# jfjlaros/HUMID

Hardware: AMD Instinct MI355X
Metric: reads/sec deduplicated, 10M PE150 UMI=8 d=1 (higher is better)
Workload: dtype u64; 1 GPU; 10000000 reads/GPU x 1 GPU (one shuffled read set of 10000000 reads, sliced by input order), PE150 UMI=8 in header -> 24-nt packed words (8+8+8), d=1, directional clustering; synthetic molecules=N/4, family 1+Geom(3), p_sub=1e-3, p_N=1e-4; reads_per_gpu=10000000, word_nt=24, distance=1, method=directional

## Files before the change

humid_amd/csrc/humid_hip.hip:

```cpp
#include "pipeline.hip.h"
#include "kernels_best.hip.h"
#include "kernels_consensus.hip.h"

static std::string g_err;
extern "C" __attribute__((visibility("hidden"))) void humid_set_global_error(const char *text) { g_err = text ? text : ""; }

extern "C" {

uint32_t humid_abi_version(void) { return HUMID_ABI_VERSION; }

int humid_device_count(void) {
  int n = 0;
  if (hipGetDeviceCount(&n) != hipSuccess) return 0;
  return n;
}

const char *humid_last_error(const humid_ctx *ctx) { return ctx ? ctx->err.c_str() : g_err.c_str(); }

int humid_ctx_create(humid_ctx **out, int device, void *stream) {
  humid_ctx *c = nullptr;
  if (!out) return fail(nullptr, HUMID_E_INVALID, "out is null");
  *out = nullptr;
  int ndev = 0;
  hipError_t e = hipGetDeviceCount(&ndev);
// ... 134 lines not shown
  }
  if (strcmp(key, "records8") == 0) {
    c->use_rec8 = value != 0;
    return HUMID_OK;
  }
  if (strcmp(key, "compact_graph") == 0) {
    c->use_compact = value != 0;
    return HUMID_OK;
  }
  if (strcmp(key, "group_buckets") == 0) {
    c->group_buckets = value != 0;
    return HUMID_OK;
  }
  if (strcmp(key, "fused_search") == 0) {
    c->fused_search = value != 0;
    return HUMID_OK;
  }
  if (strcmp(key, "padded_partition") == 0) {
    c->pt_padded = value != 0;
    return HUMID_OK;
  }
  if (strcmp(key, "force_comm") == 0) {
    c->force_comm = value != 0;
    return HUMID_OK;
  }
  if (strcmp(key, "bucket_walk") == 0) {
    if (value < 0 || value > (1 << 24)) return fail(c, HUMID_E_INVALID, "bucket_walk must be 0 (no limit) .. 2^24");
    c->walk_max = (u32)value;
    return HUMID_OK;
  }
// ... 824 lines not shown
```

humid_amd/csrc/kernels_cgraph.hip.h:

```cpp
#ifndef HUMID_KERNELS_CGRAPH_HIP_H
#define HUMID_KERNELS_CGRAPH_HIP_H

#include "common.hip.h"
#include "kernels_graph.hip.h"
#include "kernels_cluster.hip.h"

#define ER_REGIONS 64u
#define ER_STRIDE 32u
struct EdgeRegs {
  u64 *e;
  u32 cap_r;
  u32 *cur;
  const u64 *far;
  u32 n_far;
};
__device__ __forceinline__ u32 er_count(const EdgeRegs &er, u32 r) {
  if (r == ER_REGIONS) return er.n_far;
  const u32 c = er.cur[r * ER_STRIDE];
  return c < er.cap_r ? c : er.cap_r;
}
__device__ __forceinline__ u64 *er_at(const EdgeRegs &er, u32 r, u32 k) {
  return r == ER_REGIONS ? (u64 *)er.far + k : er.e + (size_t)r * er.cap_r + k;
}

// ... 31 lines not shown
static __global__ void __launch_bounds__(256)
k_bits_blocks(const u32 *__restrict__ bits, u32 n_blk, u32 *__restrict__ cnt) {
  HUMID_GUARD_LAST_VGPR();
  const u32 b = blockIdx.x * blockDim.x + threadIdx.x;
  if (b > n_blk) return;
  if (b == n_blk) { cnt[b] = 0; return; }
  const uint4 *p = (const uint4 *)(bits + 8 * (size_t)b);
  const uint4 x = p[0], y = p[1];
  cnt[b] = (u32)(__popc(x.x) + __popc(x.y) + __popc(x.z) + __popc(x.w) + __popc(y.x) + __popc(y.y) + __popc(y.z) + __popc(y.w));
}

#define ZERO_MAX 8
struct ZeroList {
  u32 *p[ZERO_MAX];
  u32 n[ZERO_MAX];
};
static __global__ void __launch_bounds__(256)
k_zero_many(ZeroList z) {
  HUMID_GUARD_LAST_VGPR();
  const u32 stride = gridDim.x * blockDim.x;
#pragma unroll
  for (u32 q = 0; q < ZERO_MAX; q++) {
    u32 *p = z.p[q];
    const u32 n = z.n[q];
    for (u32 i = blockIdx.x * blockDim.x + threadIdx.x; i < n; i += stride) p[i] = 0;
  }
}

#define PA_PPT 4u

template <class WT>
struct WordsGlobal {
  const WT *W;
  __device__ __forceinline__ WT operator()(u32 j) const { return W[j]; }
};
struct IdxSelf { __device__ __forceinline__ u32 operator()(u32 j) const { return j; } };
struct IdxGlobal {
  const u32 *V;
  __device__ __forceinline__ u32 operator()(u32 j) const { return V[j]; }
};
template <class WT>
// ... 176 lines not shown
  HUMID_GUARD_LAST_VGPR();
  const u32 r = blockIdx.y;
  const u32 n_r = er_count(er, r);
  for (u32 k = blockIdx.x * blockDim.x + threadIdx.x; k < n_r; k += gridDim.x * blockDim.x) {
    u64 *slot = er_at(er, r, k);
    const u64 e = *slot;
    const u32 a = br_rank(br, (u32)(e >> 32)), b = br_rank(br, (u32)e);
    *slot = ((u64)a << 32) | b;
    atomicAdd(&deg[a], 1u);
    atomicAdd(&deg[b], 1u);
    if (joins_for_clustering(join_by_count ? ncnt : (const u32 *)nullptr, a, b)) uf_union(parent, a, b);
  }
}

static __global__ void __launch_bounds__(256)
k_fill_and_stats(EdgeRegs er, const u32 *__restrict__ off, u32 *cur, u32 *__restrict__ idx, u32 *__restrict__ regions_max, u32 gx,
                 const u32 *__restrict__ deg, u32 *P, u32 n, u32 *csize, const u32 *__restrict__ n_dev, u32 r_first) {
  HUMID_GUARD_LAST_VGPR();
  const u32 nf = gx * (ER_REGIONS + 1 - r_first);
  if (blockIdx.x >= nf) {
    const u32 u = (blockIdx.x - nf) * blockDim.x + threadIdx.x;
    if (n_dev && *n_dev < n) n = *n_dev;
    if (u >= n || deg[u] == 0) return;
    const u32 root = uf_find(P, u);
    P[u] = root;
    atomicAdd(&csize[root], 1u);
    return;
  }
  const u32 bx = blockIdx.x % gx, r = r_first + blockIdx.x / gx;
  if (regions_max && blockIdx.x == 0 && threadIdx.x < 64) {
// ... 52 lines not shown
  if (ia >= n_ids || ib >= n_ids || ia == ib) { cpairs[k] = 0; return; }
  const u32 a = br_rank(br, ia), b = br_rank(br, ib);
  const u32 ca = (u32)r.y, cb = (u32)(r.y >> 32);
  cpairs[k] = ((u64)a << 32) | b;
  ncnt[a] = ca;
  ncnt[b] = cb;
  atomicAdd(&deg[a], 1u);
  atomicAdd(&deg[b], 1u);
  if (!join_by_count || at_least_double(ca, cb) || at_least_double(cb, ca)) uf_union(parent, a, b);
}

template <bool MAXIMUM>
__global__ void __launch_bounds__(256)
k_cg_trivial(const u32 *__restrict__ P, const u32 *__restrict__ csize, const u32 *__restrict__ m_dev, const u32 *__restrict__ cnt,
             const u32 *__restrict__ off, const u32 *__restrict__ idx, u32 *cl_of, u32 *maxleaf, u64 *cl_size, ull *ctr,
             u32 *__restrict__ small_roots) {
  HUMID_GUARD_LAST_VGPR();
  __shared__ u32 lds[4];
  __shared__ u32 lroots[CC_ROOTS], lroots_n, lroots_base;
  if (threadIdx.x == 0) lroots_n = 0;
  __syncthreads();
  const u32 n = *m_dev;
  const u32 lane = threadIdx.x & 63;
  u32 mb = 0, round = 0;
  for (u32 a0 = blockIdx.x * blockDim.x; a0 < n; a0 += gridDim.x * blockDim.x) {
    const u32 a = a0 + threadIdx.x;
    bool small_root = false;
    if (a < n) {
      const u32 root = P[a];
      const u32 members = csize[root];
      if (members > SMALL_COMP) { mb++; cl_of[a] = 0; }
      else if (members > 2) { small_root = root == a; cl_of[a] = 0; }
      else if (members == 1) { cl_of[a] = a + 1; maxleaf[a] = a; cl_size[a] = cnt[a]; }
      else if (root == a) {
        u32 b = a;
        for (u32 k = off[a]; k < off[a + 1]; k++) {
          const u32 nb = idx[k];
          if (P[nb] == root) { b = nb; break; }
        }
        const u64 ca = cnt[a], cb = cnt[b];
        if (MAXIMUM) {
          cl_of[a] = a + 1; cl_of[b] = a + 1;
          maxleaf[a] = (cb > ca) ? b : a;
          cl_size[a] = ca + cb;
        } else if (at_least_double(cb, ca)) {
          cl_of[a] = a + 1; cl_of[b] = a + 1;
          maxleaf[a] = b;
          cl_size[a] = ca + cb;
        } else if (at_least_double(ca, cb)) {
          cl_of[a] = a + 1; cl_of[b] = a + 1;
          maxleaf[a] = a;
          cl_size[a] = ca + cb;
        } else {
          cl_of[a] = a + 1; maxleaf[a] = a; cl_size[a] = ca;
          cl_of[b] = b + 1; maxleaf[b] = b; cl_size[b] = cb;
        }
      }
    }
    const u64 bm = __ballot(small_root);
    if (bm) {
      u32 base = 0;
      if (lane == 0) base = atomicAdd(&lroots_n, (u32)__popcll(bm));
      base = __shfl(base, 0);
      if (small_root) lroots[base + (u32)__popcll(bm & ((1ull << lane) - 1ull))] = a;
    }
    if ((++round & (CC_ROOTS / 256u - 1u)) == 0) {
      __syncthreads();
      const u32 cntl = lroots_n;
      if (cntl) {
        if (threadIdx.x == 0) lroots_base = (u32)atomicAdd(&ctr[CTR_SMALLROOTS], (ull)cntl);
// ... 75 lines not shown
```

humid_amd/csrc/kernels_cluster.hip.h:

```cpp
#ifndef HUMID_KERNELS_CLUSTER_HIP_H
#define HUMID_KERNELS_CLUSTER_HIP_H

#include "common.hip.h"
#include "kernels_graph.hip.h"
#include "kernels_count.hip.h"

#define MAX_CLIMB 40u

template <bool MAXIMUM, class MemberAt, class St>
__device__ __forceinline__ void cluster_one_component(MemberAt member_at, u32 n_members,
                                                      const u32 *__restrict__ cnt,
                                                      const u32 *__restrict__ off,
                                                      const u32 *__restrict__ idx, u32 *cl_of,
                                                      u32 *maxleaf, u64 *cl_size, St st) {
  for (u32 m = 0; m < n_members; m++) {
    const u32 u = member_at(m);
    if (cl_of[u] != 0) continue;
    const u32 label = u + 1;
    u32 start = u;
    u32 best = u;
    u32 bestc = 0;
    if (!MAXIMUM) {
      u32 leaf = u;
      u32 k = off[leaf], kend = off[leaf + 1];
// ... 248 lines not shown
    u32 m = k;
    while (m > 0 && mem[m - 1] > x) { mem[m] = mem[m - 1]; m--; }
    mem[m] = x;
  }
  cluster_one_component<MAXIMUM>([&](u32 m) { return mem[m]; }, nm, cnt, off, idx, cl_of, maxleaf, cl_size, st);
}

struct LdsColumn {
  u32 *base;
  __device__ __forceinline__ u32 &operator[](u32 i) const { return base[i * 64u]; }
};
template <bool MAXIMUM>
__global__ void __launch_bounds__(64)
k_cluster_small_lds(const u32 *__restrict__ roots, const ull *__restrict__ ctr, const u32 *__restrict__ P,
                    const u32 *__restrict__ csize, u32 n, const u32 *__restrict__ cnt, const u32 *__restrict__ off,
                    const u32 *__restrict__ idx, u32 *cl_of, u32 *maxleaf, u64 *cl_size) {
  HUMID_GUARD_LAST_VGPR();
  __shared__ u32 lmem[SMALL_COMP][64];
  __shared__ u32 lst[2 * SMALL_COMP][64];
  const u32 t = blockIdx.x * blockDim.x + threadIdx.x;
  if (t >= (u32)ctr[CTR_SMALLROOTS]) return;
  const u32 u = roots[t];
  if (u >= n) return;
  const u32 target = csize[u];
  if (target > SMALL_COMP || target <= 2) return;
  const LdsColumn mem{&lmem[0][threadIdx.x]}, st{&lst[0][threadIdx.x]};
  u32 nm = 1;
  mem[0] = u;
  for (u32 q = 0; q < nm && nm < target; q++) {
    const u32 v = mem[q];
    for (u32 k = off[v]; k < off[v + 1] && nm < target; k++) {
      const u32 nb = idx[k];
      bool seen = P[nb] != u;
      for (u32 j = 0; j < nm; j++) seen |= (mem[j] == nb);
      if (!seen) { mem[nm] = nb; nm++; }
    }
  }
  for (u32 k = 1; k < nm; k++) {
    const u32 x = mem[k];
    u32 m = k;
    while (m > 0 && mem[m - 1] > x) { mem[m] = mem[m - 1]; m--; }
    mem[m] = x;
  }
  cluster_one_component<MAXIMUM>([&](u32 m) { return mem[m]; }, nm, cnt, off, idx, cl_of, maxleaf, cl_size, st);
}

static __global__ void k_creator_flags(const u32 *__restrict__ cl_of, u32 n, u32 *flag) {
  HUMID_GUARD_LAST_VGPR();
  u32 u = blockIdx.x * blockDim.x + threadIdx.x;
  if (u < n) flag[u] = (cl_of[u] == u + 1) ? 1u : 0u;
}

static __global__ void k_finalize_nodes(const u32 *__restrict__ cl_of, const u32 *__restrict__ pos,
                                 const u32 *__restrict__ maxleaf, u32 n, u32 *__restrict__ cid,
                                 u8 *__restrict__ ismax, const u32 *__restrict__ s_first,
                                 const u32 *__restrict__ s_slot, u64 *__restrict__ slot_out) {
  HUMID_GUARD_LAST_VGPR();
  u32 u = blockIdx.x * blockDim.x + threadIdx.x;
  if (u >= n) return;
// ... 33 lines not shown
```

humid_amd/csrc/pipeline.hip.h:

```cpp
#ifndef HUMID_PIPELINE_HIP_H
#define HUMID_PIPELINE_HIP_H

#include <fcntl.h>
#include <sys/mman.h>
#include <sys/stat.h>
#include <unistd.h>

#include <atomic>
#include <cerrno>
#include <chrono>
#include <type_traits>
#include <utility>

#include "common.hip.h"
#include "prims.hip.h"
#include "kernels_count.hip.h"
#include "kernels_part.hip.h"
#include "kernels_part8.hip.h"
#include "kernels_graph.hip.h"
#include "kernels_cluster.hip.h"
#include "kernels_cgraph.hip.h"
#include "kernels_map.hip.h"
#include "kernels_xchg.hip.h"
#include "kernels_wide.hip.h"
// ... 54 lines not shown

struct humid_ctx {
  int device = 0;
  CtxState state;
  RunKind pass_kind = RUN_PLAIN;
  Arena arena;
  hipStream_t stream = nullptr;
  bool own_stream = false;
  std::string err;
  ull *d_ctr = nullptr;
  PsChain *ps_chain = nullptr;
  u32 ps_epoch = 0;
  ull *h_ctr = nullptr;
  ull *h_ctr_dev = nullptr;
  ull ctr_seq = 0;
  const u32 *gf_valid = nullptr;
  u32 *ucur_clean = nullptr;
  DBuf gf_cur;
  bool gf_padded = true;
  bool no_chain = false;
  bool no_poll = false;
  DBuf in_words, in_filt, in_bases, out_cid, out_keep;
  DBuf table, slot_out, slot_of_read, uniq_slot;
  DBuf pk_keys, pk_vals, pbeg, ucount, pusable, ubase, pad_word, pad_cf, pslot;
  DBuf opos, own_packed, owner, owner_sorted, perm, small;
  DBuf pc, poff, share_edges;
  DBuf own_words;
  DBuf heads;
  DBuf small_roots;
  DBuf big_runs;
// ... 13 lines not shown
  bool cg_valid = false;
  bool cg_expanded = false;
  u32 cg_M = 0, cg_nblocks = 0;
  DBuf xo_gw, xo_gc;
  DBuf xo_regs, xo_inv;
  u64 xr_ecap = 0;
  DBuf xo_send, xo_int, xo_cross, xo_sel, xo_selall, xo_parent, xo_flag, xo_xroot, xo_xcbits, xo_xcblk, xo_xcid, xo_xcall, xo_ldeg, xo_cnt;
  DBuf pw_a, pw_ai, pw_b, pw_bi;
  DBuf p8_a, p8_b, p8_cur, p8_status;
  bool use_rec8 = true;
  bool last_rec8 = false;
  const u32 *rec_cursor2 = nullptr;
  DBuf pt_work, unperm_rec, route_tiles;
  bool group_buckets = true;
  bool fused_search = true;
  bool pt_padded = true;
  bool use_tile_partition = true;
  bool last_part_tiled = false;
  int x_test_fail_after = -1, x_gathers = 0;
  bool x_hist_done = false, x_peer_failed = false;
  bool route_checked = true;
  const u32 *route_bad = nullptr;
  bool last_unperm_tiled = false;
  bool oc_valid = false, oc_fits = false;
  u32 oc_n = 0, oc_nt = 0;
  u64 oc_lo = 0, oc_scale = 0;
  u32 n_parts = 0;
  bool stage_map_timed = false;
  bool last_count_sorted = false;
  u32 g_wpr = 1;
// ... 112 lines not shown

static __global__ void k_publish_counters(const ull *__restrict__ ctr, const u32 *__restrict__ extra32, const u32 *__restrict__ extra32b,
                                   volatile ull *host, ull seq, const u32 *__restrict__ extra32c = nullptr) {
  HUMID_GUARD_LAST_VGPR();
  if (threadIdx.x < CTR_N) {
    ull v = ctr[threadIdx.x];
    if (threadIdx.x == CTR_N - 1 && extra32) v = (v & ~0xffffffffull) | (ull)*extra32;
    if (threadIdx.x == CTR_N - 2 && extra32b) v = (ull)*extra32b;
    if (threadIdx.x == CTR_N - 3 && extra32c) v = (ull)*extra32c;
    host[threadIdx.x] = v;
  }
  __threadfence_system();
  __syncthreads();
  if (threadIdx.x == 0) { host[CTR_N] = seq; __threadfence_system(); }
}
static int read_counters(humid_ctx *c, const u32 *extra32 = nullptr, const u32 *extra32b = nullptr, const u32 *extra32c = nullptr) {
  if (c->h_ctr_dev && !c->no_poll) {
    const ull seq = ++c->ctr_seq;
    hipLaunchKernelGGL(k_publish_counters, dim3(1), dim3(64), 0, c->stream, (const ull *)c->d_ctr, extra32, extra32b,
                       (volatile ull *)c->h_ctr_dev, seq, extra32c);
    HIPCHK(hipGetLastError());
    volatile ull *flag = (volatile ull *)&c->h_ctr[CTR_N];
    const auto t0 = std::chrono::steady_clock::now();
    u32 spins = 0;
    while (*flag != seq) {
      if ((++spins & 0xfffu) == 0) {
        if (hipStreamQuery(c->stream) != hipErrorNotReady) break;
        if (std::chrono::steady_clock::now() - t0 > std::chrono::seconds(30)) break;
      }
    }
    if (*flag == seq) { std::atomic_thread_fence(std::memory_order_acquire); return HUMID_OK; }
    HIPCHK(hipStreamSynchronize(c->stream));
    if (*flag == seq) return HUMID_OK;
    c->no_poll = true;
  }
  HIPCHK(hipMemcpyAsync(c->h_ctr, c->d_ctr, CTR_N * sizeof(ull), hipMemcpyDeviceToHost, c->stream));
  if (extra32)
    HIPCHK(hipMemcpyAsync(&c->h_ctr[CTR_N - 1], extra32, 4, hipMemcpyDeviceToHost, c->stream));
  if (extra32b || extra32c) {
    HIPCHK(hipStreamSynchronize(c->stream));
    if (extra32b) { c->h_ctr[CTR_N - 2] = 0; HIPCHK(hipMemcpyAsync(&c->h_ctr[CTR_N - 2], extra32b, 4, hipMemcpyDeviceToHost, c->stream)); }
    if (extra32c) { c->h_ctr[CTR_N - 3] = 0; HIPCHK(hipMemcpyAsync(&c->h_ctr[CTR_N - 3], extra32c, 4, hipMemcpyDeviceToHost, c->stream)); }
  }
  HIPCHK(hipStreamSynchronize(c->stream));
  return HUMID_OK;
}

#define TRY(...) do { int _rc = (__VA_ARGS__); if (_rc != HUMID_OK) return _rc; } while (0)

static inline void state_reset(humid_ctx *c) { c->state = CtxState{}; }
static inline void state_begin_graph(humid_ctx *c) { const bool dense = c->state.dense; state_reset(c); c->state.dense = dense; }
static inline int state_publish(humid_ctx *c, CtxState::Holds holds) {
  const bool dense = holds == CtxState::STAGE_GRAPH && c->state.dense;
  c->state = CtxState{holds, holds == CtxState::RUN ? c->pass_kind : RUN_PLAIN, dense, false};
  return HUMID_OK;
}
static inline int state_publish_count(humid_ctx *c, bool dense) { state_publish(c, CtxState::COUNT); c->state.dense = dense; return HUMID_OK; }
static inline bool state_has_leaves(const humid_ctx *c) { return c->state.holds == CtxState::RUN || c->state.holds == CtxState::STAGE_GRAPH; }
static inline bool state_has_run(const humid_ctx *c) { return c->state.holds == CtxState::RUN; }
static inline bool state_dense_count(const humid_ctx *c) { return c->state.dense; }
// ... 86 lines not shown
    }
  }
  p.ncombo = c;
  p.key_bits = maxbits;
  return p;
}

struct GraphArrays {
  u32 *deg, *parent, *csize, *off, *idx, *cl_of, *maxleaf;
  u64 *cl_size;
};
static GraphArrays legacy_arrays(humid_ctx *c) {
  return GraphArrays{c->deg.as<u32>(), c->parent.as<u32>(), c->csize.as<u32>(), c->nbr_off.as<u32>(), c->nbr_idx.as<u32>(),
                     c->cl_of.as<u32>(), c->maxleaf.as<u32>(), c->cl_size.as<u64>()};
}
static int cluster_kernels(humid_ctx *c, const GraphArrays &g, const u32 *g_cnt, u32 U, u64 M, u64 Mbig, u32 method,
                           bool trivial_done = false) {
  hipStream_t st = c->stream;
  if (!trivial_done && c->kev_on) HIPCHK(hipEventRecord(c->kev[2], st));
  if (trivial_done) {
  } else if (method == HUMID_METHOD_MAXIMUM)
    hipLaunchKernelGGL(k_cluster_trivial<true>, dim3(blocks_for(U)), dim3(256), 0, st, g.deg, g.parent, g.csize, U, g_cnt, g.off,
                       g.idx, g.cl_of, g.maxleaf, g.cl_size);
  else
    hipLaunchKernelGGL(k_cluster_trivial<false>, dim3(blocks_for(U)), dim3(256), 0, st, g.deg, g.parent, g.csize, U, g_cnt, g.off,
                       g.idx, g.cl_of, g.maxleaf, g.cl_size);
  if (M > 0) {
    const u64 small_cap = M / 3 + 1;
    if (method == HUMID_METHOD_MAXIMUM)
      hipLaunchKernelGGL(k_cluster_small_lds<true>, dim3(blocks_for(small_cap, 64)), dim3(64), 0, st, c->small_roots.as<u32>(),
                         (const ull *)c->d_ctr, g.parent, g.csize, U, g_cnt, g.off, g.idx, g.cl_of, g.maxleaf, g.cl_size);
    else
      hipLaunchKernelGGL(k_cluster_small_lds<false>, dim3(blocks_for(small_cap, 64)), dim3(64), 0, st, c->small_roots.as<u32>(),
                         (const ull *)c->d_ctr, g.parent, g.csize, U, g_cnt, g.off, g.idx, g.cl_of, g.maxleaf, g.cl_size);
    if (Mbig > 0) {
      ENSURE(c->mk0, (size_t)Mbig * 8);
      ENSURE(c->mk1, (size_t)Mbig * 8);
      ENSURE(c->stk, (size_t)Mbig * 8);
      HIPCHK(hipMemsetAsync(&c->d_ctr[CTR_SPECIAL], 0, sizeof(ull), st));
      hipLaunchKernelGGL(k_member_keys, dim3(COMPACT_BLOCKS), dim3(256), 0, st, g.deg, g.parent, g.csize, U, c->mk0.as<u64>(), c->d_ctr);
      TRY(sort_keys<u64>(c, c->mk0.as<u64>(), c->mk1.as<u64>(), Mbig, 0, 32 + bits_for(U)));
      if (method == HUMID_METHOD_MAXIMUM) {
        hipLaunchKernelGGL(k_cluster_components<true>, dim3(blocks_for(Mbig, 64)), dim3(64), 0, st,
                           c->mk1.as<u64>(), (u32)Mbig, g_cnt, g.off, g.idx, g.cl_of, g.maxleaf, g.cl_size, c->stk.as<u32>());
      } else if (c->coop_big) {
        ENSURE(c->heads, (size_t)Mbig * 4);
        HIPCHK(hipMemsetAsync(&c->d_ctr[CTR_SPECIAL], 0, sizeof(ull), st));
        hipLaunchKernelGGL(k_comp_heads, dim3(COMPACT_BLOCKS), dim3(256), 0, st, c->mk1.as<u64>(), (u32)Mbig,
                           c->heads.as<u32>(), c->d_ctr);
// ... 980 lines not shown
                     own ? c->s_slot.as<u32>() : (const u32 *)nullptr,
                     own ? c->slot_out.as<u64>() : (u64 *)nullptr);
  c->slots_done = own;
  HIPCHK(hipGetLastError());
  n_pair_segs_out = n_pair_segs;
  return HUMID_OK;
}


struct CgSource {
  EdgeRegs er;
  const ulonglong2 *recs;
  u32 n_recs;
  const RecSegs *segs = nullptr;
  const u32 *cnt_by_id;
  u32 n_ids;
  u64 pairs_bound;
};
struct CgStatus {
  bool overflow = false;
  bool group_over = false;
  u64 wanted = 0, big_mask = 0, E = 0, M = 0, Mbig = 0;
};
static GraphArrays cg_arrays(humid_ctx *c) {
  return GraphArrays{c->cg_deg.as<u32>(), c->cg_parent.as<u32>(), c->cg_csize.as<u32>(), c->cg_off.as<u32>(), c->cg_idx.as<u32>(),
                     c->cg_cl_of.as<u32>(), c->cg_maxleaf.as<u32>(), c->cg_cl_size.as<u64>()};
}
static int cg_build(humid_ctx *c, CgSource &src, u32 method, CgStatus &out) {
  hipStream_t st = c->stream;
  const u32 n_words = (((src.n_ids + 31) / 32) + 7) & ~7u, n_blk = n_words / 8;
  const u64 pb = std::max<u64>(src.pairs_bound, 1);
  if (2 * pb + 2 > 0xffffffffull) return fail(c, HUMID_E_OVERFLOW, "too many neighbour pairs");
  const u32 Mb = (u32)std::min<u64>(src.n_ids, 2 * pb);
  ENSURE(c->cg_blk, ((size_t)n_blk + 1) * 4);
  ENSURE(c->cg_nodes, ((size_t)Mb + 1) * 4);
  ENSURE(c->cg_ncnt, ((size_t)Mb + 1) * 4);
  ENSURE(c->cg_deg, ((size_t)Mb + 2) * 4);
  ENSURE(c->cg_off, ((size_t)Mb + 2) * 4);
  ENSURE(c->cg_parent, ((size_t)Mb + 1) * 4);
  ENSURE(c->cg_csize, ((size_t)Mb + 1) * 4);
  ENSURE(c->cg_curs, ((size_t)Mb + 1) * 4);
  ENSURE(c->cg_idx, (size_t)(2 * pb + 1) * 4);
  ENSURE(c->cg_cl_of, ((size_t)Mb + 1) * 4);
  ENSURE(c->cg_maxleaf, ((size_t)Mb + 1) * 4);
  ENSURE(c->cg_cl_size, ((size_t)Mb + 1) * 8);
  ENSURE(c->small_roots, ((size_t)Mb / 3 + 2) * 4);
  ENSURE(c->small, 64);
  TRY(exscan_in<u32>(c, BitsBlockIn{c->cg_bits.as<u32>(), n_blk}, c->cg_blk.as<u32>(), (u64)n_blk + 1));
  const BitRank br{c->cg_bits.as<u32>(), c->cg_blk.as<u32>()};
  const u32 *m_dev = c->cg_blk.as<u32>() + n_blk;
  const GraphArrays g = cg_arrays(c);
  hipLaunchKernelGGL(k_nodes_init, dim3(blocks_for(n_words)), dim3(256), 0, st, br, n_words, src.cnt_by_id, c->cg_nodes.as<u32>(),
                     c->cg_ncnt.as<u32>(), g.deg, g.parent, g.csize, c->cg_curs.as<u32>(), n_blk);
  const bool by_count = (method & 1) == 0;
  if (src.segs) {
    const u32 n_all = src.segs->first[REC_SEGS];
    u32 n_max = 1;
    for (u32 q = 0; q < REC_SEGS; q++) n_max = std::max(n_max, src.segs->n[q]);
    ENSURE(c->cg_far, ((size_t)n_all + 1) * 8);
    hipLaunchKernelGGL(k_segs_relabel, dim3(std::min<u32>(blocks_for(n_max), 4096), REC_SEGS), dim3(256), 0, st, *src.segs, src.n_ids, br,
                       c->cg_far.as<u64>(), c->cg_ncnt.as<u32>(), g.deg, g.parent, by_count);
    src.er.far = c->cg_far.as<u64>();
    src.er.n_far = n_all;
  } else if (src.recs) {
    ENSURE(c->cg_far, ((size_t)src.n_recs + 1) * 8);
    if (src.n_recs)
      hipLaunchKernelGGL(k_records_relabel, dim3(blocks_for(src.n_recs)), dim3(256), 0, st, src.recs, src.n_recs, src.n_ids, br,
                         c->cg_far.as<u64>(), c->cg_ncnt.as<u32>(), g.deg, g.parent, by_count);
    src.er.far = c->cg_far.as<u64>();
    src.er.n_far = src.n_recs;
  } else {
    const u32 gx = (u32)std::min<u64>(std::max<u64>(blocks_for(std::max<u64>(src.er.cap_r, src.er.n_far)), 1), 4096);
    hipLaunchKernelGGL(k_pairs_relabel, dim3(gx, ER_REGIONS + 1), dim3(256), 0, st, src.er, br, (const u32 *)c->cg_ncnt.as<u32>(),
                       g.deg, g.parent, by_count);
  }
  TRY(exscan_in<u32>(c, DegIn{g.deg, m_dev}, g.off, (u64)Mb + 1));
  {
    const u32 gx = (u32)std::min<u64>(std::max<u64>(blocks_for(std::max<u64>(src.er.cap_r, src.er.n_far)), 1), 4096);
    const u32 r_first = src.er.e ? 0u : ER_REGIONS;
    hipLaunchKernelGGL(k_fill_and_stats, dim3(gx * (ER_REGIONS + 1 - r_first) + blocks_for(Mb)), dim3(256), 0, st, src.er, (const u32 *)g.off,
                       c->cg_curs.as<u32>(), g.idx, c->small.as<u32>(), gx, (const u32 *)g.deg, g.parent, Mb, g.csize, m_dev, r_first);
  }
  hipLaunchKernelGGL(k_sort_lists, dim3(blocks_for(Mb)), dim3(256), 0, st, (const u32 *)g.off, Mb, g.idx);
  if (c->kev_on) HIPCHK(hipEventRecord(c->kev[2], st));
  const u32 tg = (u32)std::min<u64>(std::max<u64>(blocks_for(Mb), 1), 512);
  if (method == HUMID_METHOD_MAXIMUM)
    hipLaunchKernelGGL(k_cg_trivial<true>, dim3(tg), dim3(256), 0, st, (const u32 *)g.parent, (const u32 *)g.csize, m_dev,
                       (const u32 *)c->cg_ncnt.as<u32>(), (const u32 *)g.off, (const u32 *)g.idx, g.cl_of, g.maxleaf, g.cl_size, c->d_ctr,
                       c->small_roots.as<u32>());
  else
    hipLaunchKernelGGL(k_cg_trivial<false>, dim3(tg), dim3(256), 0, st, (const u32 *)g.parent, (const u32 *)g.csize, m_dev,
                       (const u32 *)c->cg_ncnt.as<u32>(), (const u32 *)g.off, (const u32 *)g.idx, g.cl_of, g.maxleaf, g.cl_size, c->d_ctr,
                       c->small_roots.as<u32>());
  HIPCHK(hipGetLastError());
  TRY(read_counters(c, g.off + Mb, c->small.as<u32>(), m_dev));
  out.wanted = (c->h_ctr[CTR_N - 2] & 0xffffffffull) * ER_REGIONS;
  out.overflow = (c->h_ctr[CTR_EOVER] & 0xffffffffull) != 0;
  out.group_over = c->h_ctr[CTR_GOVER] != 0;
  out.big_mask = c->h_ctr[CTR_BIGMASK];
  out.E = (c->h_ctr[CTR_N - 1] & 0xffffffffull) / 2;
  out.M = c->h_ctr[CTR_N - 3] & 0xffffffffull;
  out.Mbig = c->h_ctr[CTR_MEMBERS];
  return HUMID_OK;
}
static int cg_cluster_rest(humid_ctx *c, u32 n_ids, u64 M, u64 Mbig, u32 method) {
  hipStream_t st = c->stream;
  const u32 n_words = (((n_ids + 31) / 32) + 7) & ~7u, n_blk = n_words / 8;
  const GraphArrays g = cg_arrays(c);
  ENSURE(c->cg_nblk, ((size_t)n_blk + 1) * 4);
  if (M > 0) TRY(cluster_kernels(c, g, c->cg_ncnt.as<u32>(), (u32)M, M, Mbig, method, true));
  else if (c->kev_on) HIPCHK(hipEventRecord(c->kev[3], st));
  if (M > 0)
    hipLaunchKernelGGL(k_noncreator_bits, dim3(blocks_for(M)), dim3(256), 0, st, (const u32 *)g.cl_of, c->cg_nodes.as<u32>(), (u32)M,
                       c->cg_nbits.as<u32>());
  TRY(exscan_in<u32>(c, BitsBlockIn{c->cg_nbits.as<u32>(), n_blk}, c->cg_nblk.as<u32>(), (u64)n_blk + 1));
  HIPCHK(hipGetLastError());
  return HUMID_OK;
}

template <class WT>
static int stage_graph_compact(humid_ctx *c, const WT *g_word, const u32 *g_cnt, u32 U, u32 word_nt,
                               u32 distance, u32 method, humid_summary &s, u32 &n_pair_segs_out,
                               const u64 *ext_edges = nullptr, u64 n_ext_edges = 0) {
  hipStream_t st = c->stream;
  c->g_word = g_word;
  c->g_wpr = (u32)(sizeof(WT) / 8);
  c->g_cnt = g_cnt;
// ... 26 lines not shown
  CgStatus cgs;
  EdgeRegs er;
  bool ordered_seg[MAX_COMBOS] = {false};
  const u32 *seg_valid[MAX_COMBOS] = {nullptr};
  for (int attempt = 0;; attempt++) {
    if (attempt > 5) return fail(c, HUMID_E_INVALID, "internal: the pair list does not settle");
    if (search && c->cg_ecap == 0) c->cg_ecap = std::max<u64>((u64)U / 4, 4096);
    const u64 ecap = search ? c->cg_ecap : ER_REGIONS;
    if (ecap / ER_REGIONS + 1 > 0xfffffff0ull) return fail(c, HUMID_E_OVERFLOW, "too many neighbour pairs");
    er.cap_r = (u32)((ecap + ER_REGIONS - 1) / ER_REGIONS);
    ENSURE(c->cg_edges, (size_t)ER_REGIONS * er.cap_r * 8);
    er.e = c->cg_edges.as<u64>();
    er.cur = c->cg_cur.as<u32>();
    er.far = far;
    er.n_far = (u32)n_far;
    {
      ZeroList z;
      memset(&z, 0, sizeof z);
      z.p[0] = c->cg_bits.as<u32>(); z.n[0] = n_words;
      z.p[1] = c->cg_nbits.as<u32>(); z.n[1] = n_words;
      z.p[2] = c->cg_cur.as<u32>(); z.n[2] = ER_REGIONS * ER_STRIDE + 8;
      z.p[3] = (u32 *)&c->d_ctr[CTR_EDGES]; z.n[3] = 2 * (CTR_GOVER - CTR_EDGES + 1);
      hipLaunchKernelGGL(k_zero_many, dim3(64), dim3(256), 0, st, z);
    }
    auto search_alone = [&](u32 seg) -> int {
      if (seg < 8 && c->kev_on) HIPCHK(hipEventRecord(c->kev[20 + 2 * seg], st));
      pairs_append<WT>(c, ps, walked_seg<WT>(c, plan, seg, g_word, U), er, c->cg_bits.as<u32>(), &c->d_ctr[CTR_BIGMASK],
                       (u32 *)&c->d_ctr[CTR_EOVER], seg_valid[seg]);
      if (seg < 8 && c->kev_on) HIPCHK(hipEventRecord(c->kev[21 + 2 * seg], st));
      return HUMID_OK;
    };
    const bool ride_on = c->fused_search && std::is_same<WT, u64>::value;
    for (u32 seg = 0; seg < nseg; seg++) {
      bool searched = false;
      if (seg) {
        seg_valid[seg] = nullptr;
        if (!ordered_seg[seg]) {
          GroupRide ride;
// ... 3 lines not shown
              if (seg < 8 && c->kev_on) { ride.ev_group[0] = c->kev[20 + 2 * seg]; ride.ev_group[1] = c->kev[21 + 2 * seg]; }
            }
          }
          TRY(bucket_order<WT>(c, plan, seg, g_word, U, seg_ws<WT>(c, seg, U), seg_vs(c, seg, U), true, ride_on ? &ride : nullptr));
          seg_valid[seg] = c->gf_valid;
          searched = ride.did_group;
        }
        ordered_seg[seg] = true;
      }
      if (!searched) TRY(search_alone(seg));
    }
    if (n_far)
      hipLaunchKernelGGL(k_mark_pairs, dim3(blocks_for(n_far)), dim3(256), 0, st, far, (u32)n_far, U, c->cg_bits.as<u32>(), bad);
    CgSource src;
    src.er = er; src.recs = nullptr; src.n_recs = 0; src.cnt_by_id = g_cnt; src.n_ids = U;
    src.pairs_bound = ecap + n_far;
    TRY(cg_build(c, src, method, cgs));
    er = src.er;
    if (cgs.group_over) {
      c->gf_padded = false;
      for (u32 q = 0; q < MAX_COMBOS; q++) ordered_seg[q] = false;
      far = given ? ext_edges : nullptr;
      n_far = given ? n_ext_edges : 0;
      continue;
    }
    if (cgs.overflow) {
      c->cg_ecap = cgs.wanted + cgs.wanted / 2 + ER_REGIONS * 64;
      if (!given) { far = nullptr; n_far = 0; }
      continue;
    }
// ... 29 lines not shown
          ENSURE(c->cg_far, (size_t)(got + 1) * 8);
        }
      }
      far = c->cg_far.as<u64>();
      n_far = got;
      if (n_far) continue;
    }
    E = cgs.E; M = cgs.M; Mbig = cgs.Mbig;
    if (search && 2 * (cgs.wanted + cgs.wanted / 4 + ER_REGIONS * 64) < c->cg_ecap) c->cg_ecap = cgs.wanted + cgs.wanted / 4 + ER_REGIONS * 64;
    break;
  }
  s.edges = c->E = E;
  s.nonsingle = c->M = M;
  c->cg_M = (u32)M;
  if (!c->lean_events) HIPCHK(hipEventRecord(c->ev[2], st));
  TRY(cg_cluster_rest(c, U, M, Mbig, method));
  const GraphArrays g = cg_arrays(c);
  const bool own = ((const void *)g_word == c->s_word.p) && U == (u32)c->U;
  if (!own) { ENSURE(c->cid, (size_t)U * 4); ENSURE(c->ismax, (size_t)U); }
  hipLaunchKernelGGL(k_finalize_leaves, dim3(blocks_for(U)), dim3(256), 0, st, BitRank{c->cg_bits.as<u32>(), c->cg_blk.as<u32>()},
                     BitRank{c->cg_nbits.as<u32>(), c->cg_nblk.as<u32>()}, c->cg_nodes.as<u32>(), (const u32 *)g.cl_of,
                     (const u32 *)g.maxleaf, U, own ? c->s_first.as<u32>() : (const u32 *)nullptr,
                     own ? c->s_slot.as<u32>() : (const u32 *)nullptr, own ? c->slot_out.as<u64>() : (u64 *)nullptr,
                     own ? (u32 *)nullptr : c->cid.as<u32>(), own ? (u8 *)nullptr : c->ismax.as<u8>());
  c->slots_done = own;
  c->cg_valid = true;
  HIPCHK(hipGetLastError());
  n_pair_segs_out = nseg < 8 ? nseg : 8;
  return HUMID_OK;
}

// ... 582 lines not shown
```

Before: 16.53 billion reads/s.

## Fuse compact-graph node init into relabel and overlap small clustering with counter readback

Adds a default-on lean_graph path. The deg, csize and curs arrays are now zeroed, and parent filled with its identity, inside the existing zero kernel, so k_nodes_init no longer runs. Node compaction is folded into the edge relabel kernel, which also uses the original-id counts for join decisions. The small-component clustering kernel is launched (grid-stride, capped grid) between publishing and waiting on the host counter readback, and it plus the trivial kernel set the non-creator bits directly, so the separate noncreator pass can be skipped when there are no big components. This aims to remove kernel launches and a host sync bubble, at the cost of zeroing sized to a pair-count bound and extra atomics.

```diff
diff --git a/humid_amd/csrc/humid_hip.hip b/humid_amd/csrc/humid_hip.hip
--- a/humid_amd/csrc/humid_hip.hip
+++ b/humid_amd/csrc/humid_hip.hip
@@ -172,6 +172,10 @@
   }
   if (strcmp(key, "fused_search") == 0) {
     c->fused_search = value != 0;
+    return HUMID_OK;
+  }
+  if (strcmp(key, "lean_graph") == 0) {
+    c->lean_graph = value != 0;
     return HUMID_OK;
   }
   if (strcmp(key, "padded_partition") == 0) {
diff --git a/humid_amd/csrc/kernels_cgraph.hip.h b/humid_amd/csrc/kernels_cgraph.hip.h
--- a/humid_amd/csrc/kernels_cgraph.hip.h
+++ b/humid_amd/csrc/kernels_cgraph.hip.h
@@ -69,6 +69,8 @@
 struct ZeroList {
   u32 *p[ZERO_MAX];
   u32 n[ZERO_MAX];
+  u32 *iota;
+  u32 n_iota;
 };
 static __global__ void __launch_bounds__(256)
 k_zero_many(ZeroList z) {
@@ -80,6 +82,7 @@
     const u32 n = z.n[q];
     for (u32 i = blockIdx.x * blockDim.x + threadIdx.x; i < n; i += stride) p[i] = 0;
   }
+  for (u32 i = blockIdx.x * blockDim.x + threadIdx.x; i < z.n_iota; i += stride) z.iota[i] = i;
 }
 
 #define PA_PPT 4u
@@ -286,6 +289,41 @@
 }
 
 static __global__ void __launch_bounds__(256)
+k_relabel_and_nodes(EdgeRegs er, BitRank br, const u32 *__restrict__ s_cnt, u32 *deg, u32 *parent, bool join_by_count, u32 gx,
+                    u32 n_words, u32 *__restrict__ nodes, u32 *__restrict__ ncnt) {
+  HUMID_GUARD_LAST_VGPR();
+  const u32 nf = gx * (ER_REGIONS + 1);
+  if (blockIdx.x >= nf) {
+    const u32 w = (blockIdx.x - nf) * blockDim.x + threadIdx.x;
+    if (w >= n_words) return;
+    u32 x = br.bits[w];
+    if (!x) return;
+    u32 c = br_rank(br, w << 5);
+    while (x) {
+      const u32 bit = (u32)__ffs((int)x) - 1u;
+      x &= x - 1u;
+      const u32 u = (w << 5) | bit;
+      nodes[c] = u;
+      ncnt[c] = s_cnt[u];
+      c++;
+    }
+    return;
+  }
+  const u32 bx = blockIdx.x % gx, r = blockIdx.x / gx;
+  const u32 n_r = er_count(er, r);
+  for (u32 k = bx * blockDim.x + threadIdx.x; k < n_r; k += gx * blockDim.x) {
+    u64 *slot = er_at(er, r, k);
+    const u64 e = *slot;
+    const u32 ia = (u32)(e >> 32), ib = (u32)e;
+    const u32 a = br_rank(br, ia), b = br_rank(br, ib);
+    *slot = ((u64)a << 32) | b;
+    atomicAdd(&deg[a], 1u);
+    atomicAdd(&deg[b], 1u);
+    if (joins_for_clustering(join_by_count ? s_cnt : (const u32 *)nullptr, ia, ib)) uf_union(parent, a, b);
+  }
+}
+
+static __global__ void __launch_bounds__(256)
 k_fill_and_stats(EdgeRegs er, const u32 *__restrict__ off, u32 *cur, u32 *__restrict__ idx, u32 *__restrict__ regions_max, u32 gx,
                  const u32 *__restrict__ deg, u32 *P, u32 n, u32 *csize, const u32 *__restrict__ n_dev, u32 r_first) {
   HUMID_GUARD_LAST_VGPR();
@@ -368,7 +406,7 @@
 __global__ void __launch_bounds__(256)
 k_cg_trivial(const u32 *__restrict__ P, const u32 *__restrict__ csize, const u32 *__restrict__ m_dev, const u32 *__restrict__ cnt,
              const u32 *__restrict__ off, const u32 *__restrict__ idx, u32 *cl_of, u32 *maxleaf, u64 *cl_size, ull *ctr,
-             u32 *__restrict__ small_roots) {
+             u32 *__restrict__ small_roots, u32 *nc_bits, const u32 *__restrict__ nodes) {
   HUMID_GUARD_LAST_VGPR();
   __shared__ u32 lds[4];
   __shared__ u32 lroots[CC_ROOTS], lroots_n, lroots_base;
@@ -393,6 +431,7 @@
           if (P[nb] == root) { b = nb; break; }
         }
         const u64 ca = cnt[a], cb = cnt[b];
+        bool one_cluster = true;
         if (MAXIMUM) {
           cl_of[a] = a + 1; cl_of[b] = a + 1;
           maxleaf[a] = (cb > ca) ? b : a;
@@ -408,6 +447,11 @@
         } else {
           cl_of[a] = a + 1; maxleaf[a] = a; cl_size[a] = ca;
           cl_of[b] = b + 1; maxleaf[b] = b; cl_size[b] = cb;
+          one_cluster = false;
+        }
+        if (nc_bits && one_cluster && b != a) {
+          const u32 u = nodes[b];
+          atomicOr(&nc_bits[u >> 5], 1u << (u & 31));
         }
       }
     }
diff --git a/humid_amd/csrc/kernels_cluster.hip.h b/humid_amd/csrc/kernels_cluster.hip.h
--- a/humid_amd/csrc/kernels_cluster.hip.h
+++ b/humid_amd/csrc/kernels_cluster.hip.h
@@ -286,35 +286,44 @@
 __global__ void __launch_bounds__(64)
 k_cluster_small_lds(const u32 *__restrict__ roots, const ull *__restrict__ ctr, const u32 *__restrict__ P,
                     const u32 *__restrict__ csize, u32 n, const u32 *__restrict__ cnt, const u32 *__restrict__ off,
-                    const u32 *__restrict__ idx, u32 *cl_of, u32 *maxleaf, u64 *cl_size) {
+                    const u32 *__restrict__ idx, u32 *cl_of, u32 *maxleaf, u64 *cl_size, u32 *nc_bits = nullptr,
+                    const u32 *__restrict__ nodes = nullptr) {
   HUMID_GUARD_LAST_VGPR();
   __shared__ u32 lmem[SMALL_COMP][64];
   __shared__ u32 lst[2 * SMALL_COMP][64];
-  const u32 t = blockIdx.x * blockDim.x + threadIdx.x;
-  if (t >= (u32)ctr[CTR_SMALLROOTS]) return;
-  const u32 u = roots[t];
-  if (u >= n) return;
-  const u32 target = csize[u];
-  if (target > SMALL_COMP || target <= 2) return;
+  const u32 n_roots = (u32)ctr[CTR_SMALLROOTS];
   const LdsColumn mem{&lmem[0][threadIdx.x]}, st{&lst[0][threadIdx.x]};
-  u32 nm = 1;
-  mem[0] = u;
-  for (u32 q = 0; q < nm && nm < target; q++) {
-    const u32 v = mem[q];
-    for (u32 k = off[v]; k < off[v + 1] && nm < target; k++) {
-      const u32 nb = idx[k];
-      bool seen = P[nb] != u;
-      for (u32 j = 0; j < nm; j++) seen |= (mem[j] == nb);
-      if (!seen) { mem[nm] = nb; nm++; }
-    }
-  }
-  for (u32 k = 1; k < nm; k++) {
-    const u32 x = mem[k];
-    u32 m = k;
-    while (m > 0 && mem[m - 1] > x) { mem[m] = mem[m - 1]; m--; }
-    mem[m] = x;
-  }
-  cluster_one_component<MAXIMUM>([&](u32 m) { return mem[m]; }, nm, cnt, off, idx, cl_of, maxleaf, cl_size, st);
+  for (u32 t = blockIdx.x * blockDim.x + threadIdx.x; t < n_roots; t += gridDim.x * blockDim.x) {
+    const u32 u = roots[t];
+    if (u >= n) continue;
+    const u32 target = csize[u];
+    if (target > SMALL_COMP || target <= 2) continue;
+    u32 nm = 1;
+    mem[0] = u;
+    for (u32 q = 0; q < nm && nm < target; q++) {
+      const u32 v = mem[q];
+      for (u32 k = off[v]; k < off[v + 1] && nm < target; k++) {
+        const u32 nb = idx[k];
+        bool seen = P[nb] != u;
+        for (u32 j = 0; j < nm; j++) seen |= (mem[j] == nb);
+        if (!seen) { mem[nm] = nb; nm++; }
+      }
+    }
+    for (u32 k = 1; k < nm; k++) {
+      const u32 x = mem[k];
+      u32 m = k;
+      while (m > 0 && mem[m - 1] > x) { mem[m] = mem[m - 1]; m--; }
+      mem[m] = x;
+    }
+    cluster_one_component<MAXIMUM>([&](u32 m) { return mem[m]; }, nm, cnt, off, idx, cl_of, maxleaf, cl_size, st);
+    if (nc_bits)
+      for (u32 m = 0; m < nm; m++) {
+        const u32 v = mem[m];
+        if (cl_of[v] == v + 1) continue;
+        const u32 w = nodes[v];
+        atomicOr(&nc_bits[w >> 5], 1u << (w & 31));
+      }
+  }
 }
 
 static __global__ void k_creator_flags(const u32 *__restrict__ cl_of, u32 n, u32 *flag) {
diff --git a/humid_amd/csrc/pipeline.hip.h b/humid_amd/csrc/pipeline.hip.h
--- a/humid_amd/csrc/pipeline.hip.h
+++ b/humid_amd/csrc/pipeline.hip.h
@@ -92,6 +92,8 @@
   ull *h_ctr = nullptr;
   ull *h_ctr_dev = nullptr;
   ull ctr_seq = 0;
+  const u32 *ctr_extra[3] = {nullptr, nullptr, nullptr};
+  bool ctr_published = false;
   const u32 *gf_valid = nullptr;
   u32 *ucur_clean = nullptr;
   DBuf gf_cur;
@@ -135,6 +137,7 @@
   DBuf pt_work, unperm_rec, route_tiles;
   bool group_buckets = true;
   bool fused_search = true;
+  bool lean_graph = true;
   bool pt_padded = true;
   bool use_tile_partition = true;
   bool last_part_tiled = false;
@@ -277,12 +280,22 @@
   __syncthreads();
   if (threadIdx.x == 0) { host[CTR_N] = seq; __threadfence_system(); }
 }
-static int read_counters(humid_ctx *c, const u32 *extra32 = nullptr, const u32 *extra32b = nullptr, const u32 *extra32c = nullptr) {
+static int publish_counters(humid_ctx *c, const u32 *extra32 = nullptr, const u32 *extra32b = nullptr, const u32 *extra32c = nullptr) {
+  c->ctr_extra[0] = extra32; c->ctr_extra[1] = extra32b; c->ctr_extra[2] = extra32c;
+  c->ctr_published = false;
   if (c->h_ctr_dev && !c->no_poll) {
     const ull seq = ++c->ctr_seq;
     hipLaunchKernelGGL(k_publish_counters, dim3(1), dim3(64), 0, c->stream, (const ull *)c->d_ctr, extra32, extra32b,
                        (volatile ull *)c->h_ctr_dev, seq, extra32c);
     HIPCHK(hipGetLastError());
+    c->ctr_published = true;
+  }
+  return HUMID_OK;
+}
+static int wait_counters(humid_ctx *c) {
+  const u32 *extra32 = c->ctr_extra[0], *extra32b = c->ctr_extra[1], *extra32c = c->ctr_extra[2];
+  if (c->ctr_published) {
+    const ull seq = c->ctr_seq;
     volatile ull *flag = (volatile ull *)&c->h_ctr[CTR_N];
     const auto t0 = std::chrono::steady_clock::now();
     u32 spins = 0;
@@ -307,6 +320,10 @@
   }
   HIPCHK(hipStreamSynchronize(c->stream));
   return HUMID_OK;
+}
+static int read_counters(humid_ctx *c, const u32 *extra32 = nullptr, const u32 *extra32b = nullptr, const u32 *extra32c = nullptr) {
+  int rc = publish_counters(c, extra32, extra32b, extra32c);
+  return rc != HUMID_OK ? rc : wait_counters(c);
 }
 
 #define TRY(...) do { int _rc = (__VA_ARGS__); if (_rc != HUMID_OK) return _rc; } while (0)
@@ -423,8 +440,18 @@
   return GraphArrays{c->deg.as<u32>(), c->parent.as<u32>(), c->csize.as<u32>(), c->nbr_off.as<u32>(), c->nbr_idx.as<u32>(),
                      c->cl_of.as<u32>(), c->maxleaf.as<u32>(), c->cl_size.as<u64>()};
 }
+static void cluster_small(humid_ctx *c, const GraphArrays &g, const u32 *g_cnt, u32 n, u64 roots_grid, u32 method, u32 *nc_bits = nullptr,
+                          const u32 *nodes = nullptr) {
+  const u32 grid = blocks_for(roots_grid, 64);
+  if (method == HUMID_METHOD_MAXIMUM)
+    hipLaunchKernelGGL(k_cluster_small_lds<true>, dim3(grid), dim3(64), 0, c->stream, c->small_roots.as<u32>(), (const ull *)c->d_ctr,
+                       g.parent, g.csize, n, g_cnt, g.off, g.idx, g.cl_of, g.maxleaf, g.cl_size, nc_bits, nodes);
+  else
+    hipLaunchKernelGGL(k_cluster_small_lds<false>, dim3(grid), dim3(64), 0, c->stream, c->small_roots.as<u32>(), (const ull *)c->d_ctr,
+                       g.parent, g.csize, n, g_cnt, g.off, g.idx, g.cl_of, g.maxleaf, g.cl_size, nc_bits, nodes);
+}
 static int cluster_kernels(humid_ctx *c, const GraphArrays &g, const u32 *g_cnt, u32 U, u64 M, u64 Mbig, u32 method,
-                           bool trivial_done = false) {
+                           bool trivial_done = false, bool small_done = false) {
   hipStream_t st = c->stream;
   if (!trivial_done && c->kev_on) HIPCHK(hipEventRecord(c->kev[2], st));
   if (trivial_done) {
@@ -435,13 +462,7 @@
     hipLaunchKernelGGL(k_cluster_trivial<false>, dim3(blocks_for(U)), dim3(256), 0, st, g.deg, g.parent, g.csize, U, g_cnt, g.off,
                        g.idx, g.cl_of, g.maxleaf, g.cl_size);
   if (M > 0) {
-    const u64 small_cap = M / 3 + 1;
-    if (method == HUMID_METHOD_MAXIMUM)
-      hipLaunchKernelGGL(k_cluster_small_lds<true>, dim3(blocks_for(small_cap, 64)), dim3(64), 0, st, c->small_roots.as<u32>(),
-                         (const ull *)c->d_ctr, g.parent, g.csize, U, g_cnt, g.off, g.idx, g.cl_of, g.maxleaf, g.cl_size);
-    else
-      hipLaunchKernelGGL(k_cluster_small_lds<false>, dim3(blocks_for(small_cap, 64)), dim3(64), 0, st, c->small_roots.as<u32>(),
-                         (const ull *)c->d_ctr, g.parent, g.csize, U, g_cnt, g.off, g.idx, g.cl_of, g.maxleaf, g.cl_size);
+    if (!small_done) cluster_small(c, g, g_cnt, U, M / 3 + 1, method);
     if (Mbig > 0) {
       ENSURE(c->mk0, (size_t)Mbig * 8);
       ENSURE(c->mk1, (size_t)Mbig * 8);
@@ -1452,6 +1473,7 @@
   u32 n_recs;
   const RecSegs *segs = nullptr;
   const u32 *cnt_by_id;
+  bool lean = false;
   u32 n_ids;
   u64 pairs_bound;
 };
@@ -1459,6 +1481,8 @@
   bool overflow = false;
   bool group_over = false;
   u64 wanted = 0, big_mask = 0, E = 0, M = 0, Mbig = 0;
+  bool small_done = false;
+  bool bits_done = false;
 };
 static GraphArrays cg_arrays(humid_ctx *c) {
   return GraphArrays{c->cg_deg.as<u32>(), c->cg_parent.as<u32>(), c->cg_csize.as<u32>(), c->cg_off.as<u32>(), c->cg_idx.as<u32>(),
@@ -1488,8 +1512,10 @@
   const BitRank br{c->cg_bits.as<u32>(), c->cg_blk.as<u32>()};
   const u32 *m_dev = c->cg_blk.as<u32>() + n_blk;
   const GraphArrays g = cg_arrays(c);
-  hipLaunchKernelGGL(k_nodes_init, dim3(blocks_for(n_words)), dim3(256), 0, st, br, n_words, src.cnt_by_id, c->cg_nodes.as<u32>(),
-                     c->cg_ncnt.as<u32>(), g.deg, g.parent, g.csize, c->cg_curs.as<u32>(), n_blk);
+  const bool lean = src.lean && !src.segs && !src.recs && src.cnt_by_id;
+  if (!lean)
+    hipLaunchKernelGGL(k_nodes_init, dim3(blocks_for(n_words)), dim3(256), 0, st, br, n_words, src.cnt_by_id, c->cg_nodes.as<u32>(),
+                       c->cg_ncnt.as<u32>(), g.deg, g.parent, g.csize, c->cg_curs.as<u32>(), n_blk);
   const bool by_count = (method & 1) == 0;
   if (src.segs) {
     const u32 n_all = src.segs->first[REC_SEGS];
@@ -1509,8 +1535,12 @@
     src.er.n_far = src.n_recs;
   } else {
     const u32 gx = (u32)std::min<u64>(std::max<u64>(blocks_for(std::max<u64>(src.er.cap_r, src.er.n_far)), 1), 4096);
-    hipLaunchKernelGGL(k_pairs_relabel, dim3(gx, ER_REGIONS + 1), dim3(256), 0, st, src.er, br, (const u32 *)c->cg_ncnt.as<u32>(),
-                       g.deg, g.parent, by_count);
+    if (lean)
+      hipLaunchKernelGGL(k_relabel_and_nodes, dim3(gx * (ER_REGIONS + 1) + blocks_for(n_words)), dim3(256), 0, st, src.er, br, src.cnt_by_id,
+                         g.deg, g.parent, by_count, gx, n_words, c->cg_nodes.as<u32>(), c->cg_ncnt.as<u32>());
+    else
+      hipLaunchKernelGGL(k_pairs_relabel, dim3(gx, ER_REGIONS + 1), dim3(256), 0, st, src.er, br, (const u32 *)c->cg_ncnt.as<u32>(),
+                         g.deg, g.parent, by_count);
   }
   TRY(exscan_in<u32>(c, DegIn{g.deg, m_dev}, g.off, (u64)Mb + 1));
   {
@@ -1522,16 +1552,26 @@
   hipLaunchKernelGGL(k_sort_lists, dim3(blocks_for(Mb)), dim3(256), 0, st, (const u32 *)g.off, Mb, g.idx);
   if (c->kev_on) HIPCHK(hipEventRecord(c->kev[2], st));
   const u32 tg = (u32)std::min<u64>(std::max<u64>(blocks_for(Mb), 1), 512);
+  u32 *nc_bits = lean ? c->cg_nbits.as<u32>() : nullptr;
+  const u32 *nc_nodes = lean ? c->cg_nodes.as<u32>() : nullptr;
   if (method == HUMID_METHOD_MAXIMUM)
     hipLaunchKernelGGL(k_cg_trivial<true>, dim3(tg), dim3(256), 0, st, (const u32 *)g.parent, (const u32 *)g.csize, m_dev,
                        (const u32 *)c->cg_ncnt.as<u32>(), (const u32 *)g.off, (const u32 *)g.idx, g.cl_of, g.maxleaf, g.cl_size, c->d_ctr,
-                       c->small_roots.as<u32>());
+                       c->small_roots.as<u32>(), nc_bits, nc_nodes);
   else
     hipLaunchKernelGGL(k_cg_trivial<false>, dim3(tg), dim3(256), 0, st, (const u32 *)g.parent, (const u32 *)g.csize, m_dev,
                        (const u32 *)c->cg_ncnt.as<u32>(), (const u32 *)g.off, (const u32 *)g.idx, g.cl_of, g.maxleaf, g.cl_size, c->d_ctr,
-                       c->small_roots.as<u32>());
-  HIPCHK(hipGetLastError());
-  TRY(read_counters(c, g.off + Mb, c->small.as<u32>(), m_dev));
+                       c->small_roots.as<u32>(), nc_bits, nc_nodes);
+  HIPCHK(hipGetLastError());
+  TRY(publish_counters(c, g.off + Mb, c->small.as<u32>(), m_dev));
+  out.small_done = false;
+  if (lean) {
+    cluster_small(c, g, c->cg_ncnt.as<u32>(), Mb, std::min<u64>((u64)Mb / 3 + 1, 2048 * 64), method, nc_bits, nc_nodes);
+    HIPCHK(hipGetLastError());
+    out.small_done = true;
+  }
+  out.bits_done = lean;
+  TRY(wait_counters(c));
   out.wanted = (c->h_ctr[CTR_N - 2] & 0xffffffffull) * ER_REGIONS;
   out.overflow = (c->h_ctr[CTR_EOVER] & 0xffffffffull) != 0;
   out.group_over = c->h_ctr[CTR_GOVER] != 0;
@@ -1541,14 +1581,15 @@
   out.Mbig = c->h_ctr[CTR_MEMBERS];
   return HUMID_OK;
 }
-static int cg_cluster_rest(humid_ctx *c, u32 n_ids, u64 M, u64 Mbig, u32 method) {
+static int cg_cluster_rest(humid_ctx *c, u32 n_ids, u64 M, u64 Mbig, u32 method, const CgStatus *done = nullptr) {
   hipStream_t st = c->stream;
   const u32 n_words = (((n_ids + 31) / 32) + 7) & ~7u, n_blk = n_words / 8;
   const GraphArrays g = cg_arrays(c);
   ENSURE(c->cg_nblk, ((size_t)n_blk + 1) * 4);
-  if (M > 0) TRY(cluster_kernels(c, g, c->cg_ncnt.as<u32>(), (u32)M, M, Mbig, method, true));
+  const bool small_done = done && done->small_done, bits_done = done && done->bits_done;
+  if (M > 0) TRY(cluster_kernels(c, g, c->cg_ncnt.as<u32>(), (u32)M, M, Mbig, method, true, small_done));
   else if (c->kev_on) HIPCHK(hipEventRecord(c->kev[3], st));
-  if (M > 0)
+  if (M > 0 && (!bits_done || Mbig > 0))
     hipLaunchKernelGGL(k_noncreator_bits, dim3(blocks_for(M)), dim3(256), 0, st, (const u32 *)g.cl_of, c->cg_nodes.as<u32>(), (u32)M,
                        c->cg_nbits.as<u32>());
   TRY(exscan_in<u32>(c, BitsBlockIn{c->cg_nbits.as<u32>(), n_blk}, c->cg_nblk.as<u32>(), (u64)n_blk + 1));
@@ -1605,6 +1646,7 @@
     er.cur = c->cg_cur.as<u32>();
     er.far = far;
     er.n_far = (u32)n_far;
+    const bool lean = c->lean_graph;
     {
       ZeroList z;
       memset(&z, 0, sizeof z);
@@ -1612,7 +1654,22 @@
       z.p[1] = c->cg_nbits.as<u32>(); z.n[1] = n_words;
       z.p[2] = c->cg_cur.as<u32>(); z.n[2] = ER_REGIONS * ER_STRIDE + 8;
       z.p[3] = (u32 *)&c->d_ctr[CTR_EDGES]; z.n[3] = 2 * (CTR_GOVER - CTR_EDGES + 1);
-      hipLaunchKernelGGL(k_zero_many, dim3(64), dim3(256), 0, st, z);
+      u32 grid = 64;
+      if (lean) {
+        const u64 pb = std::max<u64>(ecap + n_far, 1);
+        if (2 * pb + 2 > 0xffffffffull) return fail(c, HUMID_E_OVERFLOW, "too many neighbour pairs");
+        const u32 Mb = (u32)std::min<u64>(U, 2 * pb);
+        ENSURE(c->cg_deg, ((size_t)Mb + 2) * 4);
+        ENSURE(c->cg_parent, ((size_t)Mb + 1) * 4);
+        ENSURE(c->cg_csize, ((size_t)Mb + 1) * 4);
+        ENSURE(c->cg_curs, ((size_t)Mb + 1) * 4);
+        z.p[4] = c->cg_deg.as<u32>(); z.n[4] = Mb + 1;
+        z.p[5] = c->cg_csize.as<u32>(); z.n[5] = Mb + 1;
+        z.p[6] = c->cg_curs.as<u32>(); z.n[6] = Mb + 1;
+        z.iota = c->cg_parent.as<u32>(); z.n_iota = Mb + 1;
+        grid = (u32)std::min<u64>(std::max<u64>(blocks_for((u64)Mb + 1), 64), 1024);
+      }
+      hipLaunchKernelGGL(k_zero_many, dim3(grid), dim3(256), 0, st, z);
     }
     auto search_alone = [&](u32 seg) -> int {
       if (seg < 8 && c->kev_on) HIPCHK(hipEventRecord(c->kev[20 + 2 * seg], st));
@@ -1646,6 +1703,7 @@
       hipLaunchKernelGGL(k_mark_pairs, dim3(blocks_for(n_far)), dim3(256), 0, st, far, (u32)n_far, U, c->cg_bits.as<u32>(), bad);
     CgSource src;
     src.er = er; src.recs = nullptr; src.n_recs = 0; src.cnt_by_id = g_cnt; src.n_ids = U;
+    src.lean = lean;
     src.pairs_bound = ecap + n_far;
     TRY(cg_build(c, src, method, cgs));
     er = src.er;
@@ -1705,7 +1763,7 @@
   s.nonsingle = c->M = M;
   c->cg_M = (u32)M;
   if (!c->lean_events) HIPCHK(hipEventRecord(c->ev[2], st));
-  TRY(cg_cluster_rest(c, U, M, Mbig, method));
+  TRY(cg_cluster_rest(c, U, M, Mbig, method, &cgs));
   const GraphArrays g = cg_arrays(c);
   const bool own = ((const void *)g_word == c->s_word.p) && U == (u32)c->U;
   if (!own) { ENSURE(c->cid, (size_t)U * 4); ENSURE(c->ismax, (size_t)U); }
```

Measured after the change: 16.75 billion reads/s (median of 4 runs). About the same (+1.4%).
